# 610265158/Peppa_Pig_Face_Landmark

Hardware: NVIDIA H100
Metric: faces/sec Student@256 batch=256 (higher is better)
Workload: dtype f32

## Files before the change

### peppa_pig_face_landmark_b200/csrc/conv_fpw.cu

```cuda
#include <cuda.h>
#include <cuda_fp16.h>
#include <string.h>

#include "../../include/skps_b200.h"
#include "common.h"
#include "conv_fpw.h"
#include "tc_ptx.h"

namespace skps {

constexpr int FPW_PRODUCER_REGS = 32, FPW_TRANSFORM_REGS = 160, FPW_MMA_REGS = 160;
static_assert(128 * FPW_PRODUCER_REGS + 256 * FPW_TRANSFORM_REGS + 128 * FPW_MMA_REGS <= 65536, "register file split");

__device__ __forceinline__ float2 fpw_ld2(const void* base, int fmt, long long plane, long long i) {
    if (fmt == DT_SPLIT16) {
        const __half* h = (const __half*)base;
        const float2 a = __half22float2(*reinterpret_cast<const __half2*>(h + i));
        const float2 b = __half22float2(*reinterpret_cast<const __half2*>(h + i + plane));
        return make_float2(a.x + b.x, a.y + b.y);
    }
    return *reinterpret_cast<const float2*>((const float*)base + i);
}

template <int N, int KS>
__device__ __forceinline__ void fpw_mma(float* acc, uint64_t a_hi, uint64_t a_lo, uint64_t b_hi, uint64_t b_lo,
                                        uint32_t accumulate) {
    constexpr uint64_t A_HALF = 64 * 128 >> 4;
#pragma unroll
    for (int k = 0; k < KS; ++k) {
        const uint64_t koff = (uint64_t)(k * 32 >> 4);
#pragma unroll
        for (int m = 0; m < 2; ++m)
            wg_mma3<N>(acc + (N / 2) * m, a_hi + m * A_HALF + koff, a_lo + m * A_HALF + koff, b_hi + koff, b_lo + koff,
                       k ? 1u : accumulate);
    }
}

template <int MODE, int N, int ACT, bool OUT_SPLIT>
__global__ void __launch_bounds__(XF_THREADS, 1)
conv_fpw_kernel(const __grid_constant__ CUtensorMap tm0, const __grid_constant__ CUtensorMap tm1_hi,
                const __grid_constant__ CUtensorMap tm1_lo, const __grid_constant__ CUtensorMap tmB_hi,
                const __grid_constant__ CUtensorMap tmB_lo, const __grid_constant__ CUtensorMap tmO_hi,
                const __grid_constant__ CUtensorMap tmO_lo, const __grid_constant__ CUtensorMap tmW,
                const __grid_constant__ FpwK p) {
    extern __shared__ uint8_t smem_raw[];
    __shared__ __align__(8) XfBarriers bar;

    const int warp = threadIdx.x >> 5, lane = threadIdx.x & 31;
    const uint32_t b_plane = (uint32_t)N * 128u, b_slot = 2u * b_plane;
    const XfSmem sm = xf_smem<MODE>(smem_raw, p.a, p.bs, b_slot, p.out_bufs);
    xf_cta_init<MODE>(p.a, bar, sm, smem_raw, &tm0, &tm1_hi, &tmB_hi, &tmB_lo);
    if (warp < 4) {
        asm volatile("setmaxnreg.dec.sync.aligned.u32 %0;" ::"n"(FPW_PRODUCER_REGS));
    if (warp == 0) {
        if (lane == 0) {
            int st = 0, bst = 0;
            uint32_t ph = 0, bph = 0;
            for (int u = blockIdx.x; u < p.units; u += gridDim.x) {
                const int tile = u / p.nsplit, nh = u - tile * p.nsplit;
                const int img = tile / p.a.tiles_per_img, t = tile - img * p.a.tiles_per_img;
                const int oy0 = (t / p.a.tiles_x) * XF_TH, ox0 = (t % p.a.tiles_x) * XF_TW;
                for (int kc = 0; kc < p.a.cchunks; ++kc) {
                    mbar_wait_g(smem_u32(&bar.b_empty[bst]), bph ^ 1u);
                    const uint32_t fb = smem_u32(&bar.b_full[bst]);
                    mbar_expect_tx(fb, b_slot);
                    const uint32_t dst = sm.b_off + (uint32_t)bst * b_slot;
                    tma_load_2d(dst, &tmB_hi, fb, kc * 64, nh * N);
                    tma_load_2d(dst + b_plane, &tmB_lo, fb, kc * 64, nh * N);
                    if (++bst == p.bs) { bst = 0; bph ^= 1u; }
                    xf_load_a<MODE>(p.a, bar, sm, &tm0, &tm1_hi, &tm1_lo, &tmW, kc, img, oy0, ox0, st, ph);
                }
            }
        }
    }
    } else if (warp >= 8) {
        asm volatile("setmaxnreg.inc.sync.aligned.u32 %0;" ::"n"(FPW_TRANSFORM_REGS));
        xf_transform<MODE>(p.a, bar, sm, smem_raw, p.units, [&](int u) { return u / p.nsplit; });
    } else if (warp >= 4) {
        asm volatile("setmaxnreg.inc.sync.aligned.u32 %0;" ::"n"(FPW_MMA_REGS));
        const int q = warp & 3;
        const bool leader = q == 0 && lane == 0;
        int ast = 0, bst = 0;
        uint32_t aph = 0, bph = 0;
        int store_i = 0;
        for (int u = blockIdx.x; u < p.units; u += gridDim.x) {
            const int tile = u / p.nsplit, nh = u - tile * p.nsplit;
            float acc[N];
            int prev_a = 0, prev_b = 0;
            for (int kc = 0; kc < p.a.cchunks; ++kc) {
                mbar_wait_g(smem_u32(&bar.a_full[ast]), aph);
                mbar_wait_g(smem_u32(&bar.b_full[bst]), bph);
                const uint32_t sa = sm.a_off + (uint32_t)ast * XF_A_BYTES, sb = sm.b_off + (uint32_t)bst * b_slot;
                const uint64_t a_hi = make_smem_desc(sa), a_lo = make_smem_desc(sa + XF_A_PLANE);
                const uint64_t b_hi = make_smem_desc(sb), b_lo = make_smem_desc(sb + b_plane);
                const uint32_t accumulate = kc != 0;
                wg_fence_acc(acc);
                switch (p.a.chunk_ksteps[kc]) {
                    case 4: wg_fence(); fpw_mma<N, 4>(acc, a_hi, a_lo, b_hi, b_lo, accumulate); wg_commit(); break;
                    case 3: wg_fence(); fpw_mma<N, 3>(acc, a_hi, a_lo, b_hi, b_lo, accumulate); wg_commit(); break;
                    case 2: wg_fence(); fpw_mma<N, 2>(acc, a_hi, a_lo, b_hi, b_lo, accumulate); wg_commit(); break;
                    default: wg_fence(); fpw_mma<N, 1>(acc, a_hi, a_lo, b_hi, b_lo, accumulate); wg_commit(); break;
                }
                wg_fence_acc(acc);
                wg_wait<1>();
                wg_fence_acc(acc);
                if (kc > 0 && lane == 0) {
                    mbar_arrive(smem_u32(&bar.a_empty[prev_a]));
                    mbar_arrive(smem_u32(&bar.b_empty[prev_b]));
                }
                prev_a = ast; prev_b = bst;
                if (++ast == p.a.as) { ast = 0; aph ^= 1u; }
                if (++bst == p.bs) { bst = 0; bph ^= 1u; }
            }
            wg_wait<0>();
            wg_fence_acc(acc);
            if (lane == 0) {
                mbar_arrive(smem_u32(&bar.a_empty[prev_a]));
                mbar_arrive(smem_u32(&bar.b_empty[prev_b]));
            }
// ... 141 lines not shown
    const size_t smem = xf_rings(k.a, s.mode, (size_t)L.n * 256, 0, true, k.bs, k.out_bufs);
    SKPS_CHECK(smem, "conv_fpw: layer does not fit shared memory");
    L.smem_bytes = (int)smem + 1024;
    k.Cout = s.Cout; k.out_scale = s.out_scale;
    k.bias = s.bias ? s.bias : zero_bias();
    SKPS_CHECK(k.bias, "conv_fpw: zero-bias allocation failed");
    k.res = s.res.base; k.res_fmt = s.res.fmt; k.res_plane = s.res.plane; k.res_ld = s.res.ld; k.res_coff = s.res.c_off;
    k.res_first = s.res.base ? s.res_first : 0;
    return 0;
}

template <int MODE, int N, int ACT, bool SPLIT>
static int fpw_launch_t(const FpwLayer& L, const FpwK& k, int grid, cudaStream_t stream) {
    static int attr_bytes[MAX_DEVICES] = {};
    if (smem_limit((const void*)conv_fpw_kernel<MODE, N, ACT, SPLIT>, attr_bytes, L.smem_bytes)) return 1;
    conv_fpw_kernel<MODE, N, ACT, SPLIT><<<grid, XF_THREADS, L.smem_bytes, stream>>>(
        L.src0, L.src1_hi, L.src1_lo, L.b_hi, L.b_lo, L.o_hi, L.o_lo, L.w_eff, k);
    SKPS_CUDA(cudaGetLastError());
    return 0;
}

template <int MODE, int N>
static int fpw_launch_n(const FpwLayer& L, const FpwK& k, int grid, cudaStream_t stream) {
    const bool sp = L.out_fmt == DT_SPLIT16;
    switch (L.act) {
        case ACT_NONE: return sp ? fpw_launch_t<MODE, N, ACT_NONE, true>(L, k, grid, stream) : fpw_launch_t<MODE, N, ACT_NONE, false>(L, k, grid, stream);
        case ACT_RELU: return sp ? fpw_launch_t<MODE, N, ACT_RELU, true>(L, k, grid, stream) : fpw_launch_t<MODE, N, ACT_RELU, false>(L, k, grid, stream);
        default: break;
    }
    set_error("conv_fpw: activation %d not instantiated", L.act);
    return 1;
}

Grid fpw_grid(const FpwLayer& L, int batch, int num_sms, FpwK* kp) {
    FpwK k = L.k;
    k.units = batch * k.a.tiles_per_img * k.nsplit;
    if (kp) *kp = k;
    return persistent_grid(k.units, num_sms);
}

int fpw_launch(const FpwLayer& L, int batch, int num_sms, cudaStream_t stream) {
    FpwK k;
    const int grid = fpw_grid(L, batch, num_sms, &k).ctas;
    if (L.mode == XF_DW) {
        switch (L.n) {
            case 32: return fpw_launch_n<XF_DW, 32>(L, k, grid, stream);
            case 64: return fpw_launch_n<XF_DW, 64>(L, k, grid, stream);
            default: break;
        }
    } else {
        switch (L.n) {
            case 48: return fpw_launch_n<XF_SCALE, 48>(L, k, grid, stream);
            case 64: return fpw_launch_n<XF_SCALE, 64>(L, k, grid, stream);
            default: break;
        }
    }
    set_error("conv_fpw: mode %d width %d not instantiated", L.mode, L.n);
    return 1;
}

}
```

### peppa_pig_face_landmark_b200/csrc/conv_fpw.h

```cpp
#pragma once
#include <cuda.h>
#include <cuda_runtime.h>
#include <stdint.h>

#include "xf_producer.h"

namespace skps {

struct FpwK {
    XfProducer a;
    int units;
    int nsplit;
    int bs, out_bufs;
    int Cout;
    float out_scale;
    const float* bias;
    const void* res; int res_fmt; long long res_plane; int res_ld, res_coff; int res_first;
};

struct FpwLayer {
    CUtensorMap src0, src1_hi, src1_lo, b_hi, b_lo, o_hi, o_lo, w_eff;
    FpwK k;
    int mode = 0, n = 0, act = 0, out_fmt = 0;
    int smem_bytes = 0;
};

bool fpw_supported(const XfSetup& s);
int fpw_prepare(FpwLayer& L, const XfSetup& s);
Grid fpw_grid(const FpwLayer& L, int batch, int num_sms, FpwK* k = nullptr);
int fpw_launch(const FpwLayer& L, int batch, int num_sms, cudaStream_t stream);

}
```

### peppa_pig_face_landmark_b200/csrc/debug_ops.cu

```cuda
#include <cuda_fp16.h>
#include <stdlib.h>
#include <string.h>

#include "../../include/skps_b200.h"
#include "common.h"
#include "conv_fpw.h"
#include "conv_xf.h"
#include "mpipe_kernels.h"

using namespace skps;

namespace {
struct DBuf {
    void* p = nullptr;
    ~DBuf() { if (p) cudaFree(p); }
    int put(const void* src, size_t bytes) {
        if (cudaMalloc(&p, bytes ? bytes : 16) != cudaSuccess) return 1;
        if (src && cudaMemcpy(p, src, bytes, cudaMemcpyHostToDevice) != cudaSuccess) return 1;
        return 0;
    }
};
TView mk(void* base, int C, int H, int W, int ld = 0, int fmt = DT_F32, long long plane = 0) {
    TView t;
    memset(&t, 0, sizeof(t));
// ... 19 lines not shown
    const int K = Cx + (low ? Cl : 0), Kpad = (K + 63) / 64 * 64;
    const long long nx = (long long)N * H * W * Cx, nl = low ? (long long)N * (H / 2) * (W / 2) * Cl : 0;
    const long long nout = (long long)N * H * W * Cout;
    const bool xs = x_split || mode == XF_SCALE;
    DBuf dx, dxs, dl, dg, dw, dwh, dwl, db, dr, dout, dwe;
    SKPS_CHECK(!dx.put(x, nx * 4) && !dxs.put(nullptr, nx * 4) && !dl.put(low, nl * 4) && !dg.put(gate, (size_t)N * Cx * 4) &&
               !dw.put(dww, (size_t)10 * Kpad * 4) && !dwh.put(w_hi, (size_t)n_tile * Kpad * 2) &&
               !dwl.put(w_lo, (size_t)n_tile * Kpad * 2) && !db.put(bias, (size_t)Cout * 4) && !dr.put(residual, nout * 4) &&
               !dout.put(nullptr, nout * 4 * (out_split ? 2 : 1)) && !dwe.put(weff, low ? (size_t)Cl * 144 * 4 : 0),
               "debug_conv_fused: cudaMalloc/copy failed");
    SKPS_CUDA(cudaMemcpy(dout.p, out, nout * 4, cudaMemcpyHostToDevice));
    if (xs) {
        f32_to_split<<<(unsigned)((nx + 255) / 256), 256>>>((const float*)dx.p, (__half*)dxs.p, (__half*)dxs.p + nx, nx);
        SKPS_CUDA(cudaGetLastError());
    }
    void* obase = dout.p;
    if (out_split) {
        obase = (float*)dout.p + nout;
        f32_to_split<<<(unsigned)((nout + 255) / 256), 256>>>((const float*)dout.p, (__half*)obase, (__half*)obase + nout, nout);
        SKPS_CUDA(cudaGetLastError());
    }
    XfSetup s;
    memset(&s, 0, sizeof(s));
    s.mode = mode; s.max_batch = N;
    s.x = xs ? mk(dxs.p, Cx, H, W, 0, DT_SPLIT16, nx) : mk(dx.p, Cx, H, W);
    if (low) s.low = mk(dl.p, Cl, H / 2, W / 2);
    if (gate) s.gate = mk(dg.p, Cx, 1, 1);
    s.dww = (const float*)dw.p; s.dw_act = dw_act; s.weff = low ? (const float*)dwe.p : nullptr;
    s.Cout = Cout; s.act = act; s.n_tile = n_tile; s.n_tiles = 1; s.out_scale = out_scale;
    s.w_hi = dwh.p; s.w_lo = dwl.p; s.bias = bias ? (const float*)db.p : nullptr;
    s.out = mk(obase, Cout, H, W, 0, out_split ? DT_SPLIT16 : DT_F32, nout);
    if (residual) s.res = mk(dr.p, Cout, H, W);
    s.res_first = res_first;
    if (fpw) {
        FpwLayer L;
        if (fpw_prepare(L, s) || fpw_launch(L, batch, sm_count(), 0)) return 1;
    } else {
        XfLayer L;
        if (xf_prepare(L, s) || xf_launch(L, batch, sm_count(), 0)) return 1;
    }
    SKPS_CUDA(cudaDeviceSynchronize());
    if (out_split) {
        __half* tmp = (__half*)malloc(nout * 4);
        SKPS_CHECK(tmp, "debug_conv_fused: host allocation failed");
        SKPS_CUDA(cudaMemcpy(tmp, obase, nout * 4, cudaMemcpyDeviceToHost));
        for (long long i = 0; i < nout; ++i) out[i] = __half2float(tmp[i]) + __half2float(tmp[nout + i]);
        free(tmp);
    } else {
        SKPS_CUDA(cudaMemcpy(out, dout.p, nout * 4, cudaMemcpyDeviceToHost));
    }
    return 0;
}
}

extern "C" SKPS_API int skps_debug_se_fc(const float* part, int N, int tiles, int C, const float* w1t, const float* b1,
                                         const float* w2t, const float* b2, int Cr, int act1, int act2, int hw,
                                         float* gate) {
    SKPS_CHECK(part && w1t && b1 && w2t && b2 && gate, "debug_se_fc: null argument");
    DBuf dp, dw1, db, dw2, dg;
    std::string bb((size_t)(Cr + C) * 4, '\0');
    memcpy(&bb[0], b1, (size_t)Cr * 4);
    memcpy(&bb[(size_t)Cr * 4], b2, (size_t)C * 4);
    SKPS_CHECK(!dp.put(part, (size_t)N * tiles * C * 4) && !dw1.put(w1t, (size_t)C * Cr * 4) && !db.put(bb.data(), bb.size()) &&
               !dw2.put(w2t, (size_t)C * Cr * 4) && !dg.put(nullptr, (size_t)N * C * 4), "debug_se_fc: cudaMalloc/copy failed");
    TView pv = mk(dp.p, C, tiles, 1), gv = mk(dg.p, C, 1, 1);
    if (launch_se_fc(pv, gv, (const float*)dw1.p, (const float*)db.p, (const float*)dw2.p, (const float*)db.p + Cr, Cr, act1,
                     act2, hw, N, 0))
        return 1;
    SKPS_CUDA(cudaDeviceSynchronize());
// ... 63 lines not shown
```

### peppa_pig_face_landmark_b200/csrc/engine.cu

```cuda
#include <stdarg.h>
#include <stdlib.h>
#include <string.h>

#include <map>
#include <variant>
#include <vector>

#include "../../include/skps_b200.h"
#include "common.h"
#include "conv_mma.h"
#include "conv_hm.h"
#include "conv_pw.h"
#include "conv_tc.h"
#include "conv_tct.h"
#include "conv_fpw.h"
#include "conv_xf.h"
#include "dw_tma.h"
#include "mpipe_kernels.h"
#include "stem_block.h"

namespace skps {

static thread_local char g_err[1024] = "";
void set_error(const char* fmt, ...) {
    va_list ap;
    va_start(ap, fmt);
    vsnprintf(g_err, sizeof(g_err), fmt, ap);
    va_end(ap);
}
const char* get_error() { return g_err; }

}

using namespace skps;

struct OpKernel {
    int kind = SKPS_KERNEL_MISC;
    std::variant<std::monostate, ConvMmaLayer, TcLayer, TctLayer, PwLayer, HmLayer, XfLayer, FpwLayer, DwTmaLayer,
                 UpcatTmaLayer, StemBlockW> layer;
};

struct skps_engine {
    int device = 0, max_batch = 0;
    std::vector<BufDesc> bufs;
    std::vector<void*> dbuf;
    std::vector<OpDesc> ops;
    float* d_weights = nullptr;
    std::vector<float> h_weights;
    size_t n_weights = 0;
    int input_buf = -1;
    std::vector<int> output_bufs;
    float* d_stage_f32 = nullptr;
    float* d_in_f32 = nullptr;
    bool f32_mode = false;
    std::map<int, cudaGraphExec_t> graphs;
    int launches = 0;
    bool use_graph = true;
    int device_sms = 132;
    int num_sms = 132;
    std::vector<OpKernel> kern;
    cudaStream_t s_copy = nullptr, s_compute = nullptr;
    void* d_slot_in[2] = {nullptr, nullptr};
    cudaEvent_t ev_in[2] = {nullptr, nullptr}, ev_free[2] = {nullptr, nullptr}, ev_done[2] = {nullptr, nullptr};
};

static size_t buf_elems(const BufDesc& b) { return (size_t)b.C * b.H * b.W; }
static size_t buf_bytes(const BufDesc& b) { return buf_elems(b) * (b.dtype == DT_U8 ? 1 : 4); }

static float half_bits_to_float(uint16_t h) {
    uint32_t sign = (uint32_t)(h >> 15) << 31, exp = (h >> 10) & 31, man = h & 1023, bits;
    if (exp == 0) {
        if (man == 0) { bits = sign; }
        else { int e2 = -1; do { ++e2; man <<= 1; } while (!(man & 1024)); bits = sign | ((uint32_t)(112 - e2) << 23) | ((man & 1023) << 13); }
    } else if (exp == 31) { bits = sign | 0x7F800000u | (man << 13); }
    else { bits = sign | ((exp + 112) << 23) | (man << 13); }
    float f; memcpy(&f, &bits, 4); return f;
}

static TView resolve(const skps_engine* e, const View& v) {
    TView t;
    memset(&t, 0, sizeof(t));
    if (v.buf < 0) return t;
    const BufDesc& b = e->bufs[v.buf];
    t.base = (v.buf == e->input_buf && e->f32_mode) ? (void*)e->d_in_f32 : e->dbuf[v.buf];
    t.ld = b.C;
    t.c_off = v.c_off; t.c_stride = v.c_stride; t.C = v.C; t.H = b.H; t.W = b.W;
// ... 279 lines not shown
        return 1;
    };
    if (cudaMalloc(&e->d_weights, n_floats * sizeof(float)) != cudaSuccess) { set_error("cudaMalloc weights"); return fail("alloc"); }
    if (cudaMemcpy(e->d_weights, weights, n_floats * sizeof(float), cudaMemcpyHostToDevice) != cudaSuccess) {
        set_error("cudaMemcpy weights"); return fail("copy");
    }
    for (int i = 0; i < n_bufs; ++i) {
        if (buf_elems(e->bufs[i]) * (size_t)max_batch >= ((size_t)1 << 31)) {
            set_error("buffer %d (%dx%dx%d) has 2^31 or more elements at batch %d", i, e->bufs[i].H, e->bufs[i].W,
                      e->bufs[i].C, max_batch);
            return fail("size");
        }
    }
    e->dbuf.assign(n_bufs, nullptr);
    for (int i = 0; i < n_bufs; ++i) {
        size_t bytes = buf_bytes(e->bufs[i]) * (size_t)max_batch;
        if (cudaMalloc(&e->dbuf[i], bytes ? bytes : 16) != cudaSuccess) {
            set_error("cudaMalloc buffer %d (%zu bytes)", i, bytes);
            return fail("alloc");
        }
        cudaMemset(e->dbuf[i], 0, bytes);
    }
    const BufDesc& ib = e->bufs[e->input_buf];
    if (cudaMalloc(&e->d_stage_f32, buf_elems(ib) * sizeof(float) * (size_t)max_batch) != cudaSuccess ||
        cudaMalloc(&e->d_in_f32, buf_elems(ib) * sizeof(float) * (size_t)max_batch) != cudaSuccess) {
        set_error("cudaMalloc staging");
        return fail("alloc");
    }
    cudaDeviceGetAttribute(&e->device_sms, cudaDevAttrMultiProcessorCount, device);
    e->num_sms = e->device_sms;
    e->kern.resize(n_ops);
    for (int i = 0; i < n_ops; ++i)
        if (const char* what = prepare_op(e, i)) return fail(what);
    *out = e;
    return 0;
}

extern "C" SKPS_API void skps_engine_destroy(skps_engine* e) {
    if (!e) return;
    DeviceGuard on(e->device);
    for (auto& kv : e->graphs) cudaGraphExecDestroy(kv.second);
    for (void* p : e->dbuf) if (p) cudaFree(p);
    for (int i = 0; i < 2; ++i) {
        if (e->d_slot_in[i]) cudaFree(e->d_slot_in[i]);
        if (e->ev_in[i]) cudaEventDestroy(e->ev_in[i]);
        if (e->ev_free[i]) cudaEventDestroy(e->ev_free[i]);
        if (e->ev_done[i]) cudaEventDestroy(e->ev_done[i]);
    }
    if (e->s_copy) cudaStreamDestroy(e->s_copy);
    if (e->s_compute) cudaStreamDestroy(e->s_compute);
    if (e->d_weights) cudaFree(e->d_weights);
    if (e->d_stage_f32) cudaFree(e->d_stage_f32);
    if (e->d_in_f32) cudaFree(e->d_in_f32);
    delete e;
}

extern "C" SKPS_API int skps_engine_input_dims(const skps_engine* e, int* h, int* w, int* c) {
    SKPS_CHECK(e, "null engine");
    const BufDesc& b = e->bufs[e->input_buf];
    if (h) *h = b.H;
    if (w) *w = b.W;
    if (c) *c = b.C;
    return 0;
}
extern "C" SKPS_API int skps_engine_num_outputs(const skps_engine* e) { return e ? (int)e->output_bufs.size() : 0; }
extern "C" SKPS_API int skps_engine_output_elems(const skps_engine* e, int idx) {
    if (!e || idx < 0 || idx >= (int)e->output_bufs.size()) return 0;
    return (int)buf_elems(e->bufs[e->output_bufs[idx]]);
}
extern "C" SKPS_API void* skps_engine_input_ptr(skps_engine* e) { return e ? e->dbuf[e->input_buf] : nullptr; }
extern "C" SKPS_API float* skps_engine_output_ptr(skps_engine* e, int idx) {
    if (!e || idx < 0 || idx >= (int)e->output_bufs.size()) return nullptr;
    return (float*)e->dbuf[e->output_bufs[idx]];
}
extern "C" SKPS_API int skps_engine_num_buffers(const skps_engine* e) { return e ? (int)e->bufs.size() : 0; }
extern "C" SKPS_API int skps_engine_buffer_dims(const skps_engine* e, int buf, int* h, int* w, int* c, int* dtype) {
    SKPS_CHECK(e && buf >= 0 && buf < (int)e->bufs.size(), "buffer_dims: bad index");
    const BufDesc& b = e->bufs[buf];
    if (h) *h = b.H;
    if (w) *w = b.W;
    if (c) *c = b.C;
    if (dtype) *dtype = b.dtype;
    return 0;
}
extern "C" SKPS_API int skps_engine_read_buffer(skps_engine* e, int buf, int batch, void* dst) {
    SKPS_CHECK(e && buf >= 0 && buf < (int)e->bufs.size() && batch <= e->max_batch, "read_buffer: bad arguments");
// ... 229 lines not shown
```

### peppa_pig_face_landmark_b200/csrc/xf_producer.h

```cpp
#pragma once
#include <cuda.h>
#include <cuda_fp16.h>
#include <cuda_runtime.h>
#include <stdint.h>

#include "common.h"
#include "tc_ptx.h"

namespace skps {

enum { XF_SCALE = 0, XF_DW = 1 };
enum { XS_UP_F32 = 0, XS_DW_F32 = 1, XS_DW_SPLIT = 2 };
constexpr int XF_MAX_CHUNKS = 16;

constexpr int XF_THREADS = 512;
constexpr int XF_TW = 16, XF_TH = 8;
constexpr int XF_IW = XF_TW + 2, XF_IH = XF_TH + 2;
constexpr int XF_LW = XF_TW / 2 + 2, XF_LH = XF_TH / 2 + 2;
constexpr int XF_RAW_BYTES = XF_IH * XF_IW * 128;
constexpr int XF_UP_BYTES = XF_LH * XF_LW * 128;
constexpr int XF_A_PLANE = 128 * 128;
constexpr int XF_A_BYTES = 2 * XF_A_PLANE;
constexpr int XF_RING = 4;
constexpr int XF_OUT_BUF = 16384;
// ... 7 lines not shown
    int dw_act;
    int Cout, act, n_tile, n_tiles;
    float out_scale;
    const void* w_hi; const void* w_lo;
    const float* bias;
    TView out, res;
    int res_first;
};

struct XfProducer {
    int H, W, tiles_x, tiles_per_img;
    int cchunks, Cin;
    int rs, as;
    int dw_act;
    int Hl, Wl;
    int halves;
    int wcx;
    uint8_t sub_mode[2 * XF_MAX_CHUNKS];
    int16_t sub_c[2 * XF_MAX_CHUNKS];
    uint8_t chunk_subs[XF_MAX_CHUNKS];
    uint8_t chunk_ksteps[XF_MAX_CHUNKS];
    const float* dww;
    const float* gate; int gate_ld, gate_coff;
};

bool xf_supported(const XfSetup& s);
int xf_producer_prepare(XfProducer& k, CUtensorMap& src0, CUtensorMap& src1_hi, CUtensorMap& src1_lo, CUtensorMap& w_eff,
                        const XfSetup& s);
size_t xf_rings(XfProducer& k, int mode, size_t b_slot, size_t reserve, bool two_out_bufs, int& bs, int& out_bufs);

struct XfBarriers {
    uint64_t raw_full[XF_RING], raw_empty[XF_RING], a_raw[XF_RING], a_full[XF_RING], a_empty[XF_RING], b_full[XF_RING],
        b_empty[XF_RING];
};

struct XfSmem {
    uint32_t a_off, b_off, o_off, r_off, w_off;
};

template <int MODE>
__device__ __forceinline__ XfSmem xf_smem(const uint8_t* smem_raw, const XfProducer& p, int bs, uint32_t b_slot, int out_bufs) {
    XfSmem s;
    s.a_off = (smem_u32(smem_raw) + 1023u) & ~1023u;
    s.b_off = s.a_off + (uint32_t)p.as * XF_A_BYTES;
    s.o_off = s.b_off + (uint32_t)bs * b_slot;
    s.r_off = s.o_off + (uint32_t)out_bufs * XF_OUT_BUF;
    s.w_off = s.r_off + (MODE == XF_DW ? (uint32_t)p.rs * XF_RAW_BYTES : 0u);
    return s;
}

template <int MODE>
__device__ __forceinline__ void xf_cta_init(const XfProducer& p, XfBarriers& bar, const XfSmem& sm, uint8_t* smem_raw,
                                            const CUtensorMap* tm0, const CUtensorMap* tm1_hi, const CUtensorMap* tmB_hi,
                                            const CUtensorMap* tmB_lo) {
    const int warp = threadIdx.x >> 5, lane = threadIdx.x & 31;
    if (warp == 0 && lane == 0) {
        asm volatile("prefetch.tensormap [%0];" ::"l"(tm0) : "memory");
        asm volatile("prefetch.tensormap [%0];" ::"l"(tm1_hi) : "memory");
        asm volatile("prefetch.tensormap [%0];" ::"l"(tmB_hi) : "memory");
        asm volatile("prefetch.tensormap [%0];" ::"l"(tmB_lo) : "memory");
    }
    if (warp == 1 && lane == 0) {
        for (int s = 0; s < XF_RING; ++s) {
            mbar_init(smem_u32(&bar.raw_full[s]), 1);
            mbar_init(smem_u32(&bar.raw_empty[s]), p.halves ? 4 : 8);
            mbar_init(smem_u32(&bar.a_raw[s]), 1);
            mbar_init(smem_u32(&bar.a_full[s]), 8);
            mbar_init(smem_u32(&bar.a_empty[s]), 4);
            mbar_init(smem_u32(&bar.b_full[s]), 1);
            mbar_init(smem_u32(&bar.b_empty[s]), 4);
        }
        asm volatile("fence.mbarrier_init.release.cluster;" ::: "memory");
    }
    if (MODE == XF_DW) {
        float* dws = reinterpret_cast<float*>(smem_raw + (sm.w_off - smem_u32(smem_raw)));
        for (int i = threadIdx.x; i < 10 * p.cchunks * 64; i += XF_THREADS) dws[i] = __ldg(p.dww + i);
    }
    __syncthreads();
}

template <int MODE>
__device__ __forceinline__ void xf_load_a(const XfProducer& p, XfBarriers& bar, const XfSmem& sm, const CUtensorMap* tm0,
                                          const CUtensorMap* tm1_hi, const CUtensorMap* tm1_lo, const CUtensorMap* tmW,
                                          int kc, int img, int oy0, int ox0, int& st, uint32_t& ph) {
    if (MODE == XF_SCALE) {
        mbar_wait_g(smem_u32(&bar.a_empty[st]), ph ^ 1u);
        const uint32_t fb = smem_u32(&bar.a_raw[st]);
        mbar_expect_tx(fb, XF_A_BYTES);
        const uint32_t dst = sm.a_off + (uint32_t)st * XF_A_BYTES;
        tma_load_4d(dst, tm1_hi, fb, kc * 64, ox0, oy0, img);
        tma_load_4d(dst + XF_A_PLANE, tm1_lo, fb, kc * 64, ox0, oy0, img);
        if (++st == p.as) { st = 0; ph ^= 1u; }
        return;
    }
    const int subs = p.chunk_subs[kc];
    for (int h = 0; h < subs; ++h) {
        const int si = kc * 2 + h, smode = p.sub_mode[si], c = p.sub_c[si];
        mbar_wait_g(smem_u32(&bar.raw_empty[st]), ph ^ 1u);
        const uint32_t fb = smem_u32(&bar.raw_full[st]);
        const uint32_t dst = sm.r_off + (uint32_t)st * XF_RAW_BYTES;
        if (smode == XS_UP_F32) {
            mbar_expect_tx(fb, XF_UP_BYTES + (uint32_t)p.wcx * 3u * 9u * 128u);
            tma_load_4d(dst, tm0, fb, c, (ox0 >> 1) - 1, (oy0 >> 1) - 1, img);
            tma_load_5d(dst + XF_UP_BYTES, tmW, fb, 0, 0, (p.wcx == 4 || ox0 == 0) ? 0 : 1, oy0 == 0 ? 0 : 1, c >> 5);
// ... 1 lines not shown
            mbar_expect_tx(fb, XF_RAW_BYTES);
            tma_load_4d(dst, tm0, fb, c, ox0 - 1, oy0 - 1, img);
        } else {
            mbar_expect_tx(fb, XF_RAW_BYTES);
            tma_load_4d(dst, tm1_hi, fb, c, ox0 - 1, oy0 - 1, img);
            tma_load_4d(dst + XF_RAW_BYTES / 2, tm1_lo, fb, c, ox0 - 1, oy0 - 1, img);
        }
        if (++st == p.rs) { st = 0; ph ^= 1u; }
    }
}

__device__ __forceinline__ void split_store4(uint32_t addr_hi, const float4 v) {
    const __half2 h01 = __floats2half2_rn(v.x, v.y), h23 = __floats2half2_rn(v.z, v.w);
    const float2 f01 = __half22float2(h01), f23 = __half22float2(h23);
    const __half2 l01 = __floats2half2_rn(v.x - f01.x, v.y - f01.y), l23 = __floats2half2_rn(v.z - f23.x, v.w - f23.y);
    asm volatile("st.shared.v2.b32 [%0], {%1, %2};" ::"r"(addr_hi), "r"(*reinterpret_cast<const uint32_t*>(&h01)),
                 "r"(*reinterpret_cast<const uint32_t*>(&h23)) : "memory");
    asm volatile("st.shared.v2.b32 [%0], {%1, %2};" ::"r"(addr_hi + (uint32_t)XF_A_PLANE),
                 "r"(*reinterpret_cast<const uint32_t*>(&l01)), "r"(*reinterpret_cast<const uint32_t*>(&l23)) : "memory");
}
__device__ __forceinline__ float4 f4_fma(const float4 a, const float4 w, const float4 c) {
    return make_float4(fmaf(a.x, w.x, c.x), fmaf(a.y, w.y, c.y), fmaf(a.z, w.z, c.z), fmaf(a.w, w.w, c.w));
}

template <int ACT>
__device__ __forceinline__ void act16(float4* acc) {
#pragma unroll
    for (int q = 0; q < 4; ++q) {
        acc[q].x = act_t<ACT>(acc[q].x); acc[q].y = act_t<ACT>(acc[q].y);
        acc[q].z = act_t<ACT>(acc[q].z); acc[q].w = act_t<ACT>(acc[q].w);
    }
}

template <int MODE, class TileOf>
__device__ __forceinline__ void xf_transform(const XfProducer& p, XfBarriers& bar, const XfSmem& sm, uint8_t* smem_raw,
                                             int n_work, TileOf tile_of) {
    const int lane = threadIdx.x & 31;
    const int tt = threadIdx.x - 256;
    const int Kpad = p.cchunks * 64;
    int ast = 0, rst = 0;
    uint32_t aph = 0, rph = 0;
    if (MODE == XF_SCALE) {
        const int r0 = tt >> 3, ps = tt & 7, j = ps ^ (r0 & 7);
        for (int u = blockIdx.x; u < n_work; u += gridDim.x) {
            const int img = tile_of(u) / p.tiles_per_img;
            const float* grow = p.gate + (long long)img * p.gate_ld + p.gate_coff;
            for (int kc = 0; kc < p.cchunks; ++kc) {
                const int c = kc * 64 + j * 8;
                float g[8];
                if (c < p.Cin) {
                    const float4 g0 = __ldg(reinterpret_cast<const float4*>(grow + c));
                    const float4 g1 = __ldg(reinterpret_cast<const float4*>(grow + c + 4));
                    g[0] = g0.x; g[1] = g0.y; g[2] = g0.z; g[3] = g0.w; g[4] = g1.x; g[5] = g1.y; g[6] = g1.z; g[7] = g1.w;
                } else {
#pragma unroll
                    for (int e = 0; e < 8; ++e) g[e] = 0.f;
                }
                mbar_wait_g(smem_u32(&bar.a_raw[ast]), aph);
                const uint32_t sa = sm.a_off + (uint32_t)ast * XF_A_BYTES + (uint32_t)ps * 16u;
#pragma unroll
                for (int i = 0; i < 4; ++i) {
                    const uint32_t ad = sa + (uint32_t)(r0 + 32 * i) * 128u;
                    uint32_t hv[4], lv[4];
                    asm volatile("ld.shared.v4.b32 {%0, %1, %2, %3}, [%4];" : "=r"(hv[0]), "=r"(hv[1]), "=r"(hv[2]), "=r"(hv[3]) : "r"(ad) : "memory");
                    asm volatile("ld.shared.v4.b32 {%0, %1, %2, %3}, [%4];" : "=r"(lv[0]), "=r"(lv[1]), "=r"(lv[2]), "=r"(lv[3]) : "r"(ad + (uint32_t)XF_A_PLANE) : "memory");
#pragma unroll
                    for (int e = 0; e < 4; ++e) {
                        const float2 hf = __half22float2(*reinterpret_cast<const __half2*>(&hv[e]));
                        const float2 lf = __half22float2(*reinterpret_cast<const __half2*>(&lv[e]));
                        const float v0 = (hf.x + lf.x) * g[2 * e], v1 = (hf.y + lf.y) * g[2 * e + 1];
                        const __half2 h2 = __floats2half2_rn(v0, v1);
                        const float2 h2f = __half22float2(h2);
                        const __half2 l2 = __floats2half2_rn(v0 - h2f.x, v1 - h2f.y);
                        hv[e] = *reinterpret_cast<const uint32_t*>(&h2);
// ... 42 lines not shown
                                    in[i] = make_float4(a01.x + b01.x, a01.y + b01.y, a23.x + b23.x, a23.y + b23.y);
                                }
                            }
#pragma unroll
                            for (int kx = 0; kx < 3; ++kx) {
                                const float4 w = *reinterpret_cast<const float4*>(dws + (ky * 3 + kx) * Kpad + cw);
#pragma unroll
                                for (int q = 0; q < 4; ++q) acc[q] = f4_fma(in[q + kx], w, acc[q]);
                            }
                        }
                    }
                    __syncwarp();
                    if (lane == 0) mbar_arrive(smem_u32(&bar.raw_empty[rst]));
                    if (++rst == p.rs) { rst = 0; rph ^= 1u; }
                    const int jc = h * 4 + (cl >> 1);
                    switch (p.dw_act) {
                        case ACT_RELU: act16<ACT_RELU>(acc); break;
                        case ACT_HSWISH: act16<ACT_HSWISH>(acc); break;
                        case ACT_SILU: act16<ACT_SILU>(acc); break;
                        default: break;
                    }
#pragma unroll
                    for (int q = 0; q < 4; ++q) {
                        const float4 v = acc[q];
                        const int r = prow * XF_TW + xs + q;
                        split_store4(sa + (uint32_t)r * 128u + (uint32_t)((jc ^ (r & 7)) << 4) + (uint32_t)(cl & 1) * 8u, v);
                    }
                }
                asm volatile("fence.proxy.async.shared::cta;" ::: "memory");
                __syncwarp();
                if (lane == 0) mbar_arrive(smem_u32(&bar.a_full[ast]));
                if (++ast == p.as) { ast = 0; aph ^= 1u; }
            }
        }
    } else {
        const int half = tt >> 7, t7 = tt & 127;
        const int cl = t7 & 7, pg = t7 >> 3, xs = (pg & 3) * 4, rp = pg >> 2;
        const float* dws = reinterpret_cast<const float*>(smem_raw + (sm.w_off - smem_u32(smem_raw)));
        for (int u = blockIdx.x; u < n_work; u += gridDim.x) {
            const int t = tile_of(u) % p.tiles_per_img;
            const int oy0 = (t / p.tiles_x) * XF_TH, ox0 = (t % p.tiles_x) * XF_TW;
            const int ox = ox0 + xs;
            for (int kc = 0; kc < p.cchunks; ++kc) {
                mbar_wait_g(smem_u32(&bar.a_empty[ast]), aph ^ 1u);
                const uint32_t sa = sm.a_off + (uint32_t)ast * XF_A_BYTES;
                const int subs = p.chunk_subs[kc];
                if (half < subs) {
                    int slot = rst + half;
                    uint32_t sph = rph;
                    if (slot >= p.rs) { slot -= p.rs; sph ^= 1u; }
                    const int smode = p.sub_mode[kc * 2 + half];
                    const int cw = kc * 64 + half * 32 + cl * 4;
                    const float4 bias4 = *reinterpret_cast<const float4*>(dws + 9 * Kpad + cw);
                    float4 acc[2][4] = {{bias4, bias4, bias4, bias4}, {bias4, bias4, bias4, bias4}};
                    int r0, r1;
                    mbar_wait_g(smem_u32(&bar.raw_full[slot]), sph);
                    const uint8_t* raw = smem_raw + (sm.r_off + (uint32_t)slot * XF_RAW_BYTES - smem_u32(smem_raw));
                    if (smode == XS_UP_F32) {
                        r0 = (rp >> 1) * 4 + (rp & 1); r1 = r0 + 2;
                        const int y0 = oy0 + r0, y1 = oy0 + r1;
                        const int ly0 = (oy0 >> 1) - 1, lx0 = (ox0 >> 1) - 1, m = y0 >> 1, c2 = ox >> 1;
                        const int cyb = oy0 == 0 ? 0 : 1, cxb = (p.wcx == 4 || ox0 == 0) ? 0 : 1;
                        const int cyA = (y0 == 0 ? 0 : (y0 == p.H - 1 ? 3 : 1 + (y0 & 1))) - cyb;
                        const int cyB = (y1 == 0 ? 0 : (y1 == p.H - 1 ? 3 : 1 + (y1 & 1))) - cyb;
                        const bool same_cy = cyA == cyB;
                        const bool xfirst = ox == 0, xlast = ox + 4 == p.W;
// ... 73 lines not shown
                                if (wr > 0) {
                                    const float4 x = wprev[kx];
#pragma unroll
                                    for (int q = 0; q < 4; ++q) acc[1][q] = f4_fma(in[q + kx], x, acc[1][q]);
                                }
                                wprev[kx] = w;
                            }
                        }
                    }
                    __syncwarp();
                    if (lane == 0) mbar_arrive(smem_u32(&bar.raw_empty[slot]));
                    switch (p.dw_act) {
                        case ACT_RELU: act16<ACT_RELU>(acc[0]); act16<ACT_RELU>(acc[1]); break;
                        case ACT_HSWISH: act16<ACT_HSWISH>(acc[0]); act16<ACT_HSWISH>(acc[1]); break;
                        case ACT_SILU: act16<ACT_SILU>(acc[0]); act16<ACT_SILU>(acc[1]); break;
                        default: break;
                    }
                    const int jc = half * 4 + (cl >> 1);
#pragma unroll
                    for (int rr = 0; rr < 2; ++rr)
#pragma unroll
                        for (int q = 0; q < 4; ++q) {
                            const int r = (rr ? r1 : r0) * XF_TW + xs + q;
                            split_store4(sa + (uint32_t)r * 128u + (uint32_t)((jc ^ (r & 7)) << 4) + (uint32_t)(cl & 1) * 8u, acc[rr][q]);
                        }
                }
                rst += subs;
                if (rst >= p.rs) { rst -= p.rs; rph ^= 1u; }
                asm volatile("fence.proxy.async.shared::cta;" ::: "memory");
                __syncwarp();
                if (lane == 0) mbar_arrive(smem_u32(&bar.a_full[ast]));
                if (++ast == p.as) { ast = 0; aph ^= 1u; }
            }
        }
    }
}

}
```

Baseline: 20110.

## Reuse transformed depthwise A tiles across N-splits via global scratch reloads

In depthwise mode with split output channels, each tile is now processed once per CTA for all N-splits. The first pass saves the transformed A operand to a per-CTA global scratch buffer with bulk copies. Later passes reload it by TMA bulk copy instead of re-running the depthwise transform and input loads. This removes duplicated depthwise compute and input traffic, at the cost of extra global writes and reads, new barriers and warps, and coarser work items that can leave the persistent grid less evenly balanced.

Result: faster. 20610, median of 6 (+2.5%).

```diff
diff --git a/peppa_pig_face_landmark_b200/csrc/conv_fpw.cu b/peppa_pig_face_landmark_b200/csrc/conv_fpw.cu
--- a/peppa_pig_face_landmark_b200/csrc/conv_fpw.cu
+++ b/peppa_pig_face_landmark_b200/csrc/conv_fpw.cu
@@ -34,6 +34,17 @@
             wg_mma3<N>(acc + (N / 2) * m, a_hi + m * A_HALF + koff, a_lo + m * A_HALF + koff, b_hi + koff, b_lo + koff,
                        k ? 1u : accumulate);
     }
+}
+
+__device__ __forceinline__ int fpw_grid_ctas() {
+    int n;
+    asm volatile("mov.u32 %0, %%nctaid.x;" : "=r"(n));
+    return n;
+}
+
+template <int MODE>
+__device__ __forceinline__ int fpw_per_item(const FpwK& p) {
+    return MODE == XF_DW && p.a.halves ? p.nsplit : 1;
 }
 
 template <int MODE, int N, int ACT, bool OUT_SPLIT>
@@ -49,15 +60,19 @@
     const int warp = threadIdx.x >> 5, lane = threadIdx.x & 31;
     const uint32_t b_plane = (uint32_t)N * 128u, b_slot = 2u * b_plane;
     const XfSmem sm = xf_smem<MODE>(smem_raw, p.a, p.bs, b_slot, p.out_bufs);
-    xf_cta_init<MODE>(p.a, bar, sm, smem_raw, &tm0, &tm1_hi, &tmB_hi, &tmB_lo);
+    const int per_item = fpw_per_item<MODE>(p);
+    const bool reuse = per_item > 1;
+    uint8_t* const scratch = reuse ? p.scratch + (size_t)blockIdx.x * p.a.cchunks * XF_A_BYTES : nullptr;
+    xf_cta_init<MODE>(p.a, bar, sm, smem_raw, &tm0, &tm1_hi, &tmB_hi, &tmB_lo, reuse ? 5 : 4);
     if (warp < 4) {
         asm volatile("setmaxnreg.dec.sync.aligned.u32 %0;" ::"n"(FPW_PRODUCER_REGS));
     if (warp == 0) {
         if (lane == 0) {
             int st = 0, bst = 0;
             uint32_t ph = 0, bph = 0;
-            for (int u = blockIdx.x; u < p.units; u += gridDim.x) {
-                const int tile = u / p.nsplit, nh = u - tile * p.nsplit;
+            for (int w = blockIdx.x, j = 0; w < p.items; j = j + 1 < fpw_per_item<MODE>(p) ? j + 1 : 0, w += j ? 0 : fpw_grid_ctas()) {
+                const bool tiles = fpw_per_item<MODE>(p) > 1;
+                const int tile = tiles ? w : w / p.nsplit, nh = tiles ? j : w - tile * p.nsplit;
                 const int img = tile / p.a.tiles_per_img, t = tile - img * p.a.tiles_per_img;
                 const int oy0 = (t / p.a.tiles_x) * XF_TH, ox0 = (t % p.a.tiles_x) * XF_TW;
                 for (int kc = 0; kc < p.a.cchunks; ++kc) {
@@ -68,14 +83,63 @@
                     tma_load_2d(dst, &tmB_hi, fb, kc * 64, nh * N);
                     tma_load_2d(dst + b_plane, &tmB_lo, fb, kc * 64, nh * N);
                     if (++bst == p.bs) { bst = 0; bph ^= 1u; }
-                    xf_load_a<MODE>(p.a, bar, sm, &tm0, &tm1_hi, &tm1_lo, &tmW, kc, img, oy0, ox0, st, ph);
+                    if (j == 0)
+                        xf_load_a<MODE>(p.a, bar, sm, &tm0, &tm1_hi, &tm1_lo, &tmW, kc, img, oy0, ox0, st, ph);
                 }
             }
+        }
+    } else if (warp == 1) {
+        if (reuse && lane == 0) {
+            int ast = 0;
+            uint32_t aph = 0;
+            for (int w = blockIdx.x; w < p.items; w += gridDim.x)
+                for (int j = 0; j < per_item; ++j)
+                    for (int kc = 0; kc < p.a.cchunks; ++kc) {
+                        mbar_wait_g(smem_u32(&bar.a_full[ast]), aph);
+                        if (j == 0) {
+                            asm volatile("cp.async.bulk.global.shared::cta.bulk_group [%0], [%1], %2;"
+                                         ::"l"(scratch + (size_t)kc * XF_A_BYTES), "r"(sm.a_off + (uint32_t)ast * XF_A_BYTES),
+                                         "r"((uint32_t)XF_A_BYTES) : "memory");
+                            asm volatile("cp.async.bulk.commit_group;" ::: "memory");
+                            asm volatile("cp.async.bulk.wait_group.read 0;" ::: "memory");
+                        }
+                        mbar_arrive(smem_u32(&bar.a_empty[ast]));
+                        if (++ast == p.a.as) { ast = 0; aph ^= 1u; }
+                        if (j == 0 && kc == p.a.cchunks - 1) {
+                            asm volatile("cp.async.bulk.wait_group 0;" ::: "memory");
+                            asm volatile("fence.proxy.async.global;" ::: "memory");
+                            mbar_arrive(smem_u32(&bar.a_saved));
+                        }
+                    }
+        }
+    } else if (warp == 2) {
+        if (reuse && lane == 0) {
+            int ast = 0;
+            uint32_t aph = 0, saved_ph = 0;
+            for (int w = blockIdx.x; w < p.items; w += gridDim.x)
+                for (int j = 0; j < per_item; ++j)
+                    for (int kc = 0; kc < p.a.cchunks; ++kc) {
+                        if (j > 0) {
+                            if (j == 1 && kc == 0) {
+                                mbar_wait_g(smem_u32(&bar.a_saved), saved_ph);
+                                saved_ph ^= 1u;
+                                asm volatile("fence.proxy.async.global;" ::: "memory");
+                            }
+                            mbar_wait_g(smem_u32(&bar.a_empty[ast]), aph ^ 1u);
+                            const uint32_t ab = smem_u32(&bar.a_raw[ast]);
+                            mbar_expect_tx(ab, XF_A_BYTES);
+                            asm volatile("cp.async.bulk.shared::cluster.global.mbarrier::complete_tx::bytes [%0], [%1], %2, [%3];"
+                                         ::"r"(sm.a_off + (uint32_t)ast * XF_A_BYTES), "l"(scratch + (size_t)kc * XF_A_BYTES),
+                                         "r"((uint32_t)XF_A_BYTES), "r"(ab) : "memory");
+                        }
+                        if (++ast == p.a.as) { ast = 0; aph ^= 1u; }
+                    }
         }
     }
     } else if (warp >= 8) {
         asm volatile("setmaxnreg.inc.sync.aligned.u32 %0;" ::"n"(FPW_TRANSFORM_REGS));
-        xf_transform<MODE>(p.a, bar, sm, smem_raw, p.units, [&](int u) { return u / p.nsplit; });
+        xf_transform<MODE>(p.a, bar, sm, smem_raw, p.items, [&](int w) { return per_item > 1 ? w : w / p.nsplit; },
+                           per_item);
     } else if (warp >= 4) {
         asm volatile("setmaxnreg.inc.sync.aligned.u32 %0;" ::"n"(FPW_MMA_REGS));
         const int q = warp & 3;
@@ -83,8 +147,10 @@
         int ast = 0, bst = 0;
         uint32_t aph = 0, bph = 0;
         int store_i = 0;
-        for (int u = blockIdx.x; u < p.units; u += gridDim.x) {
-            const int tile = u / p.nsplit, nh = u - tile * p.nsplit;
+        for (int w = blockIdx.x; w < p.items; w += gridDim.x)
+        for (int j = 0; j < fpw_per_item<MODE>(p); ++j) {
+            const bool tiles = fpw_per_item<MODE>(p) > 1;
+            const int tile = tiles ? w : w / p.nsplit, nh = tiles ? j : w - tile * p.nsplit;
             float acc[N];
             int prev_a = 0, prev_b = 0;
             for (int kc = 0; kc < p.a.cchunks; ++kc) {
@@ -292,16 +358,22 @@
     return 1;
 }
 
+size_t fpw_scratch_per_cta(const FpwLayer& L) {
+    return L.mode == XF_DW && L.k.a.halves && L.k.nsplit > 1 ? (size_t)L.k.a.cchunks * XF_A_BYTES : 0;
+}
+
 Grid fpw_grid(const FpwLayer& L, int batch, int num_sms, FpwK* kp) {
     FpwK k = L.k;
-    k.units = batch * k.a.tiles_per_img * k.nsplit;
+    k.items = batch * k.a.tiles_per_img * (fpw_scratch_per_cta(L) ? 1 : k.nsplit);
     if (kp) *kp = k;
-    return persistent_grid(k.units, num_sms);
+    return persistent_grid(k.items, num_sms);
 }
 
 int fpw_launch(const FpwLayer& L, int batch, int num_sms, cudaStream_t stream) {
     FpwK k;
     const int grid = fpw_grid(L, batch, num_sms, &k).ctas;
+    SKPS_CHECK(!fpw_scratch_per_cta(L) || (k.scratch && grid <= L.scratch_ctas),
+               "conv_fpw: A-tile scratch for %d CTAs, launch of %d", k.scratch ? L.scratch_ctas : 0, grid);
     if (L.mode == XF_DW) {
         switch (L.n) {
             case 32: return fpw_launch_n<XF_DW, 32>(L, k, grid, stream);
diff --git a/peppa_pig_face_landmark_b200/csrc/conv_fpw.h b/peppa_pig_face_landmark_b200/csrc/conv_fpw.h
--- a/peppa_pig_face_landmark_b200/csrc/conv_fpw.h
+++ b/peppa_pig_face_landmark_b200/csrc/conv_fpw.h
@@ -9,8 +9,9 @@
 
 struct FpwK {
     XfProducer a;
-    int units;
+    int items;
     int nsplit;
+    uint8_t* scratch;
     int bs, out_bufs;
     int Cout;
     float out_scale;
@@ -23,10 +24,12 @@
     FpwK k;
     int mode = 0, n = 0, act = 0, out_fmt = 0;
     int smem_bytes = 0;
+    int scratch_ctas = 0;
 };
 
 bool fpw_supported(const XfSetup& s);
 int fpw_prepare(FpwLayer& L, const XfSetup& s);
+size_t fpw_scratch_per_cta(const FpwLayer& L);
 Grid fpw_grid(const FpwLayer& L, int batch, int num_sms, FpwK* k = nullptr);
 int fpw_launch(const FpwLayer& L, int batch, int num_sms, cudaStream_t stream);
 
diff --git a/peppa_pig_face_landmark_b200/csrc/debug_ops.cu b/peppa_pig_face_landmark_b200/csrc/debug_ops.cu
--- a/peppa_pig_face_landmark_b200/csrc/debug_ops.cu
+++ b/peppa_pig_face_landmark_b200/csrc/debug_ops.cu
@@ -75,9 +75,17 @@
     s.out = mk(obase, Cout, H, W, 0, out_split ? DT_SPLIT16 : DT_F32, nout);
     if (residual) s.res = mk(dr.p, Cout, H, W);
     s.res_first = res_first;
+    DBuf scratch;
     if (fpw) {
         FpwLayer L;
-        if (fpw_prepare(L, s) || fpw_launch(L, batch, sm_count(), 0)) return 1;
+        if (fpw_prepare(L, s)) return 1;
+        const int sms = sm_count();
+        if (const size_t per_cta = fpw_scratch_per_cta(L)) {
+            SKPS_CHECK(!scratch.put(nullptr, per_cta * sms), "debug_conv_fused: cudaMalloc failed");
+            L.k.scratch = (uint8_t*)scratch.p;
+            L.scratch_ctas = sms;
+        }
+        if (fpw_launch(L, batch, sms, 0)) return 1;
     } else {
         XfLayer L;
         if (xf_prepare(L, s) || xf_launch(L, batch, sm_count(), 0)) return 1;
diff --git a/peppa_pig_face_landmark_b200/csrc/engine.cu b/peppa_pig_face_landmark_b200/csrc/engine.cu
--- a/peppa_pig_face_landmark_b200/csrc/engine.cu
+++ b/peppa_pig_face_landmark_b200/csrc/engine.cu
@@ -2,6 +2,7 @@
 #include <stdlib.h>
 #include <string.h>
 
+#include <algorithm>
 #include <map>
 #include <variant>
 #include <vector>
@@ -52,6 +53,7 @@
     std::vector<int> output_bufs;
     float* d_stage_f32 = nullptr;
     float* d_in_f32 = nullptr;
+    void* d_fpw_scratch = nullptr;
     bool f32_mode = false;
     std::map<int, cudaGraphExec_t> graphs;
     int launches = 0;
@@ -397,6 +399,21 @@
     e->kern.resize(n_ops);
     for (int i = 0; i < n_ops; ++i)
         if (const char* what = prepare_op(e, i)) return fail(what);
+    size_t per_cta = 0;
+    for (const OpKernel& k : e->kern)
+        if (k.kind == SKPS_KERNEL_FPW) per_cta = std::max(per_cta, fpw_scratch_per_cta(std::get<FpwLayer>(k.layer)));
+    if (per_cta) {
+        if (cudaMalloc(&e->d_fpw_scratch, per_cta * e->device_sms) != cudaSuccess) {
+            set_error("cudaMalloc conv_fpw scratch (%zu bytes)", per_cta * e->device_sms);
+            return fail("alloc");
+        }
+        for (OpKernel& k : e->kern)
+            if (k.kind == SKPS_KERNEL_FPW) {
+                FpwLayer& L = std::get<FpwLayer>(k.layer);
+                L.k.scratch = (uint8_t*)e->d_fpw_scratch;
+                L.scratch_ctas = e->device_sms;
+            }
+    }
     *out = e;
     return 0;
 }
@@ -417,6 +434,7 @@
     if (e->d_weights) cudaFree(e->d_weights);
     if (e->d_stage_f32) cudaFree(e->d_stage_f32);
     if (e->d_in_f32) cudaFree(e->d_in_f32);
+    if (e->d_fpw_scratch) cudaFree(e->d_fpw_scratch);
     delete e;
 }
 
diff --git a/peppa_pig_face_landmark_b200/csrc/xf_producer.h b/peppa_pig_face_landmark_b200/csrc/xf_producer.h
--- a/peppa_pig_face_landmark_b200/csrc/xf_producer.h
+++ b/peppa_pig_face_landmark_b200/csrc/xf_producer.h
@@ -63,6 +63,7 @@
 struct XfBarriers {
     uint64_t raw_full[XF_RING], raw_empty[XF_RING], a_raw[XF_RING], a_full[XF_RING], a_empty[XF_RING], b_full[XF_RING],
         b_empty[XF_RING];
+    uint64_t a_saved;
 };
 
 struct XfSmem {
@@ -83,7 +84,7 @@
 template <int MODE>
 __device__ __forceinline__ void xf_cta_init(const XfProducer& p, XfBarriers& bar, const XfSmem& sm, uint8_t* smem_raw,
                                             const CUtensorMap* tm0, const CUtensorMap* tm1_hi, const CUtensorMap* tmB_hi,
-                                            const CUtensorMap* tmB_lo) {
+                                            const CUtensorMap* tmB_lo, int a_readers = 4) {
     const int warp = threadIdx.x >> 5, lane = threadIdx.x & 31;
     if (warp == 0 && lane == 0) {
         asm volatile("prefetch.tensormap [%0];" ::"l"(tm0) : "memory");
@@ -97,10 +98,11 @@
             mbar_init(smem_u32(&bar.raw_empty[s]), p.halves ? 4 : 8);
             mbar_init(smem_u32(&bar.a_raw[s]), 1);
             mbar_init(smem_u32(&bar.a_full[s]), 8);
-            mbar_init(smem_u32(&bar.a_empty[s]), 4);
+            mbar_init(smem_u32(&bar.a_empty[s]), a_readers);
             mbar_init(smem_u32(&bar.b_full[s]), 1);
             mbar_init(smem_u32(&bar.b_empty[s]), 4);
         }
+        mbar_init(smem_u32(&bar.a_saved), 1);
         asm volatile("fence.mbarrier_init.release.cluster;" ::: "memory");
     }
     if (MODE == XF_DW) {
@@ -168,14 +170,25 @@
     }
 }
 
+__device__ __forceinline__ void xf_take_reloads(const XfProducer& p, XfBarriers& bar, int reloads, int& ast, uint32_t& aph,
+                                                uint32_t& a_raw_par) {
+    for (int i = 0; i < reloads * p.cchunks; ++i) {
+        mbar_wait_g(smem_u32(&bar.a_raw[ast]), (a_raw_par >> ast) & 1u);
+        a_raw_par ^= 1u << ast;
+        __syncwarp();
+        if ((threadIdx.x & 31) == 0) mbar_arrive(smem_u32(&bar.a_full[ast]));
+        if (++ast == p.as) { ast = 0; aph ^= 1u; }
+    }
+}
+
 template <int MODE, class TileOf>
 __device__ __forceinline__ void xf_transform(const XfProducer& p, XfBarriers& bar, const XfSmem& sm, uint8_t* smem_raw,
-                                             int n_work, TileOf tile_of) {
+                                             int n_work, TileOf tile_of, int reps = 1) {
     const int lane = threadIdx.x & 31;
     const int tt = threadIdx.x - 256;
     const int Kpad = p.cchunks * 64;
     int ast = 0, rst = 0;
-    uint32_t aph = 0, rph = 0;
+    uint32_t aph = 0, rph = 0, a_raw_par = 0;
     if (MODE == XF_SCALE) {
         const int r0 = tt >> 3, ps = tt & 7, j = ps ^ (r0 & 7);
         for (int u = blockIdx.x; u < n_work; u += gridDim.x) {
@@ -284,6 +297,7 @@
                 if (lane == 0) mbar_arrive(smem_u32(&bar.a_full[ast]));
                 if (++ast == p.as) { ast = 0; aph ^= 1u; }
             }
+            xf_take_reloads(p, bar, reps - 1, ast, aph, a_raw_par);
         }
     } else {
         const int half = tt >> 7, t7 = tt & 127;
@@ -423,6 +437,7 @@
                 if (lane == 0) mbar_arrive(smem_u32(&bar.a_full[ast]));
                 if (++ast == p.as) { ast = 0; aph ^= 1u; }
             }
+            xf_take_reloads(p, bar, reps - 1, ast, aph, a_raw_par);
         }
     }
 }
```
